# mateomarin/two_towers

Hardware: AMD Instinct MI355X
Metric: training pairs/sec at global batch=8192, 1/2/4/8 GPUs; MRR@10 match (higher is better)
Workload: dtype bf16; 1 GPU; BASELINE configs[2]: EnhancedTwoTowerModel(300, 256), seq_len 64, batch 8192 per GPU, bf16, hard-negative mining k=5 + margin 0.2, dropout 0.1, Adam; global_batch=8192, seq_len=64, hidden=256, embedding_dim=300, parallelism=dp1, loss=hardneg_margin

## Files before the change

two_towers_amd/csrc/tt_gemm.hip:

```cpp
#include <float.h>
#include <stdarg.h>
#include <stdlib.h>

#include <atomic>
#include <type_traits>

#include "tt_api.h"
#include "tt_gemm_core.h"

namespace tt {
static thread_local char g_err[512];
void set_error(const char* fmt, ...) {
  va_list ap;
  va_start(ap, fmt);
  vsnprintf(g_err, sizeof(g_err), fmt, ap);
  va_end(ap);
}
}

namespace tt {
namespace {
struct OptDef {
  const char* name;
  const char* env;
// ... 109 lines not shown
  using ML = std::conditional_t<
      DMA,
      std::conditional_t<TBM == 256 && TBN == 256 && WGM == 2 && WGN == 4,
                         ttg::Loop8<T, AKO, BKO, TT_GEMM_BAL, A3, false, BUF>,
                         ttg::DLoop<T, AKO, BKO, TBM, TBN, WGM, WGN>>,
      ttg::MainLoop<T, AKO, BKO, TBM, TBN>>;
  static_assert(DMA || (TBM == 128 && TBN == 128 && WGM == 2 && WGN == 2), "register path is 128x128");
  constexpr int NT = 64 * WGM * WGN;
  constexpr int LDSB = ML::LDS_BYTES > 64 * (TBN + 4) * 4 ? ML::LDS_BYTES : 64 * (TBN + 4) * 4;
  __shared__ __attribute__((aligned(16))) char lds[LDSB];
  const int ntn = (g.N + TBN - 1) / TBN, ntm = (g.M + TBM - 1) / TBM;
  const int id = xcd_remap(blockIdx.x, gridDim.x);
  const int bs = id / (ntm * ntn), tile = id - bs * (ntm * ntn);
  const int mt = tile / ntn, nt = tile - mt * ntn;
  const int bi = bs / g.splits, s = bs - bi * g.splits;
  const int m0 = mt * TBM, n0 = nt * TBN;
  const T* A = static_cast<const T*>(g.a[bi]);
  const T* B = static_cast<const T*>(g.b[bi]);

  f32x4 acc[ML::TM][ML::TN];
#pragma unroll
  for (int i = 0; i < ML::TM; ++i)
#pragma unroll
    for (int j = 0; j < ML::TN; ++j) acc[i][j] = f32x4{0.f, 0.f, 0.f, 0.f};

  const int nk = (g.K * (int)sizeof(T) + ttg::KTB - 1) / ttg::KTB;
  const int kt0 = s * g.kt_per_split;
  const int kt1 = min(nk, kt0 + g.kt_per_split);

  constexpr bool L8T = DMA && TBM == 256 && TBN == 256 && WGM == 2 && WGN == 4;
  const bool mm = !L8T || !TT_TAIL_SKIP || __builtin_amdgcn_readfirstlane((int)(m0 + (int)(threadIdx.x >> 8) * 128 < g.M));
  auto lrun = [&](const auto& la, const auto& lb) {
    if constexpr (L8T) ML::run(la, lb, g.K, kt0, kt1, lds, acc, mm);
    else ML::run(la, lb, g.K, kt0, kt1, lds, acc);
  };
  auto run = [&](const auto& la) {
    if constexpr (!BKO) {
      lrun(la, ttg::KCPlain<T>{B, g.ldb, n0, g.N});
    } else if constexpr (SHIFT) {
      lrun(la, ttg::KOShift<T>{B, g.ldb, n0, g.N - n0, g.seq_t, g.bshift[bi]});
    } else {
      lrun(la, ttg::KOPlain<T>{B, g.ldb, n0, g.N - n0});
    }
  };
  if constexpr (AKO) {
    ttg::KOPlain<T> la{A, g.lda, m0, g.M - m0};
    if (g.a_split > 0) {
      la.base1 = static_cast<const T*>(g.a_hi[bi]);
      la.csplit = g.a_split;
    }
    run(la);
  } else {
    run(ttg::KCPlain<T>{A, g.lda, m0, g.M});
  }

#ifdef TT_DIAG
  if (g.force_regstage == 9) {
    float sum = 0.f;
#pragma unroll
    for (int i = 0; i < ML::TM; ++i)
#pragma unroll
      for (int j = 0; j < ML::TN; ++j) sum += acc[i][j][0] + acc[i][j][3];
    if (sum == 12345.f) static_cast<float*>(g.c[bi])[0] = 1.f;
    return;
  }
#endif
  const bool partial = g.splits > 1;
  TO* C = partial ? nullptr : static_cast<TO*>(g.c[bi]);
  float* P = partial ? static_cast<float*>(g.c[bi]) + (long)s * g.part_stride : nullptr;
  const long ldc = partial ? (long)g.N : g.ldc;
  const float* bias = partial ? nullptr : g.bias[bi];
  const int wave = threadIdx.x >> 6, lane = threadIdx.x & 63, tid = threadIdx.x;
  constexpr int WTM = TBM / WGM, WTN = TBN / WGN;
  const int wm = wave / WGN * WTM, wn = wave % WGN * WTN;
  constexpr int CLD = TBN + 4;
  constexpr int TPR = TBN / 8;
  constexpr int RPP = NT / TPR;
  float* L = reinterpret_cast<float*>(lds);
  const int cg = (tid % TPR) * 8;
  const __amdgpu_buffer_rsrc_t crs = tt_rsrc(partial ? (const void*)P : (const void*)(C + (long)m0 * ldc + n0));
  float bv[8];
#pragma unroll
  for (int e = 0; e < 8; ++e) bv[e] = 0.f;
  if (bias) {
    if (n0 + cg + 8 <= g.N && g.bias_vec_ok) ld8(bias + n0 + cg, bv);
    else
      for (int e = 0; e < 8; ++e)
        if (n0 + cg + e < g.N) bv[e] = bias[n0 + cg + e];
  }
  for (int hf = 0; hf < TBM / 64; ++hf) {
    if (wm <= hf * 64 && hf * 64 < wm + WTM) {
      const int i0 = (hf * 64 - wm) / 16;
#pragma unroll
      for (int i = 0; i < ML::TM; ++i)
        if (i >= i0 && i < i0 + 4)
#pragma unroll
          for (int j = 0; j < ML::TN; ++j)
#pragma unroll
            for (int r = 0; r < 4; ++r)
              L[(16 * (i - i0) + 4 * (lane >> 4) + r) * CLD + wn + 16 * j + (lane & 15)] = acc[i][j][r];
    }
    __syncthreads();
#pragma unroll
    for (int k = 0; k < 64 / RPP; ++k) {
      const int rl = tid / TPR + RPP * k;
      const int gm = m0 + hf * 64 + rl, gn = n0 + cg;
      if (gm < g.M && gn < g.N) {
        float v[8];
#pragma unroll
        for (int e = 0; e < 8; ++e) v[e] = L[rl * CLD + cg + e];
        const bool full = gn + 8 <= g.N && g.vec_ok;
        if (partial) {
          float* dst = P + (long)gm * ldc + gn;
          if (full) st8(dst, v);
          else
            for (int e = 0; e < 8 && gn + e < g.N; ++e) dst[e] = v[e];
        } else {
#pragma unroll
          for (int e = 0; e < 8; ++e) {
            float x = v[e] * g.alpha + bv[e];
            if (g.relu) x = fmaxf(x, 0.f);
            if (g.drop_thresh) x *= tt_dropout_scale(g.drop_seed, g.drop_row0 + (uint32_t)gm, gn + e, g.drop_thresh, g.drop_inv_keep);
            v[e] = x;
          }
          TO* dst = C + (long)gm * ldc + gn;
          if (full) {
            if (g.beta) {
              float o[8];
              ld8(dst, o);
#pragma unroll
              for (int e = 0; e < 8; ++e) v[e] += o[e];
            }
            if (g.stream_out)
              st8_sc1(crs, (int)(((long)(gm - m0) * ldc + (gn - n0)) * (long)sizeof(TO)), v, (TO*)nullptr);
            else
              st8(dst, v);
          } else {
            for (int e = 0; e < 8 && gn + e < g.N; ++e) {
              float x = v[e];
              if (g.beta) x += Elt<TO>::ld(dst + e);
              Elt<TO>::st(dst + e, x);
            }
          }
        }
      }
    }
    __syncthreads();
  }
}

template <typename TO>
constexpr int EPI_STORES = sizeof(TO) == 2 ? 16 : 32;

template <typename TO, int MI = -1, int NI = -1>
TT_DEV void epi_direct(const GemmArgs& g, const f32x4 (&acc)[8][4], TO* C, const float* bias, int m0, int n0,
                       int wm, int wn, bool full) {
  constexpr int I0 = MI < 0 ? 0 : 4 * MI, I1 = MI < 0 ? 8 : 4 * MI + 4;
  constexpr int JP0 = NI < 0 ? 0 : NI, JP1 = NI < 0 ? 2 : NI + 1;
  const int lane = threadIdx.x & 63, q = lane >> 4, lr = lane & 15;
  float bv[4][4];
#pragma unroll
  for (int j = 0; j < 4; ++j)
#pragma unroll
    for (int e = 0; e < 4; ++e) bv[j][e] = 0.f;
  if (bias) {
#pragma unroll
    for (int j = 2 * JP0; j < 2 * JP1; ++j) {
      const int c = n0 + wn + 16 * j + 4 * q;
      if (full && g.bias_vec_ok) {
        const float4 b4 = *reinterpret_cast<const float4*>(bias + c);
        bv[j][0] = b4.x; bv[j][1] = b4.y; bv[j][2] = b4.z; bv[j][3] = b4.w;
      } else {
        for (int e = 0; e < 4; ++e)
          if (c + e < g.N) bv[j][e] = bias[c + e];
      }
    }
  }
#ifdef TT_DIAG
  if (g.force_regstage == 9) {
    float sum = 0.f;
#pragma unroll
    for (int i = 0; i < 8; ++i)
#pragma unroll
      for (int j = 0; j < 4; ++j) sum += acc[i][j][0] + acc[i][j][3] + bv[j][0];
    if (sum == 12345.f) C[0] = (TO)0;
    return;
  }
#endif
  const __amdgpu_buffer_rsrc_t crs = tt_rsrc(C + (long)m0 * g.ldc + n0);
  auto fin = [&](float x, float b, int gm, int gn) {
    x = x * g.alpha + b;
    if (g.relu) x = fmaxf(x, 0.f);
    if (g.drop_thresh) x *= tt_dropout_scale(g.drop_seed, g.drop_row0 + (uint32_t)gm, gn, g.drop_thresh, g.drop_inv_keep);
    return x;
  };
  auto put = [&](int gm, int gn, uint4 v) {
#ifdef TT_DIAG
    if (g.force_regstage == 10) {
      *reinterpret_cast<uint4*>(C + (long)(gm & 63) * g.ldc + gn) = v;
      return;
    }
#endif
    const int off = (int)(((long)(gm - m0) * g.ldc + (gn - n0)) * (long)sizeof(TO));
    if (g.stream_out == 2) st16_buf_aux<2>(crs, off, v);
    else if (g.stream_out == 3) st16_buf_aux<17>(crs, off, v);
    else if (g.stream_out) st16_sc1(crs, off, v);
    else *reinterpret_cast<uint4*>(C + (long)gm * g.ldc + gn) = v;
  };
#pragma unroll
  for (int i = I0; i < I1; ++i) {
    const int gm = m0 + wm + 16 * i + lr;
    if constexpr (sizeof(TO) == 2) {
#if TT_EPI_PAIR
      if (NI < 0 && full) {
        uint4 v[2];
#pragma unroll
        for (int jp = 0; jp < 2; ++jp) {
          uint32_t w[2][2];
#pragma unroll
          for (int h = 0; h < 2; ++h) {
            const int j = 2 * jp + h, c = n0 + wn + 16 * j + 4 * q;
            float x[4];
#pragma unroll
            for (int e = 0; e < 4; ++e) x[e] = fin(acc[i][j][e], bv[j][e], gm, c + e);
            w[h][0] = (uint32_t)f2bf(x[0]) | ((uint32_t)f2bf(x[1]) << 16);
            w[h][1] = (uint32_t)f2bf(x[2]) | ((uint32_t)f2bf(x[3]) << 16);
          }
          const auto s0 = __builtin_amdgcn_permlane16_swap(w[0][0], w[1][0], false, false);
          const auto s1 = __builtin_amdgcn_permlane16_swap(w[0][1], w[1][1], false, false);
          v[jp] = make_uint4(s0[0], s1[0], s0[1], s1[1]);
        }
        uint4 da, db;
        row_pair(v[0], v[1], da, db);
        const int ra = m0 + wm + 16 * i + (lr & 7);
        const int cs = n0 + wn + 16 * (q & 1) + 8 * (q >> 1) + (lr & 8 ? 32 : 0);
        put(ra, cs, da);
        put(ra + 8, cs, db);
        continue;
      }
#endif
#pragma unroll
      for (int jp = JP0; jp < JP1; ++jp) {
        uint32_t w[2][2];
#pragma unroll
        for (int h = 0; h < 2; ++h) {
          const int j = 2 * jp + h, c = n0 + wn + 16 * j + 4 * q;
          float v[4];
#pragma unroll
          for (int e = 0; e < 4; ++e) v[e] = fin(acc[i][j][e], bv[j][e], gm, c + e);
          w[h][0] = (uint32_t)f2bf(v[0]) | ((uint32_t)f2bf(v[1]) << 16);
          w[h][1] = (uint32_t)f2bf(v[2]) | ((uint32_t)f2bf(v[3]) << 16);
        }
        const auto s0 = __builtin_amdgcn_permlane16_swap(w[0][0], w[1][0], false, false);
        const auto s1 = __builtin_amdgcn_permlane16_swap(w[0][1], w[1][1], false, false);
        const uint4 v = make_uint4(s0[0], s1[0], s0[1], s1[1]);
        const int cs = n0 + wn + 16 * (2 * jp + (q & 1)) + 8 * (q >> 1);
        if (full) {
          put(gm, cs, v);
        } else if (gm < g.M) {
          if (cs + 8 <= g.N && g.vec_ok) {
            put(gm, cs, v);
          } else {
            const uint32_t u[4] = {v.x, v.y, v.z, v.w};
            for (int e = 0; e < 8 && cs + e < g.N; ++e)
              Elt<TO>::st(C + (long)gm * g.ldc + cs + e, __uint_as_float(e & 1 ? u[e >> 1] & 0xFFFF0000u : u[e >> 1] << 16));
          }
        }
      }
    } else {
#pragma unroll
      for (int j = 2 * JP0; j < 2 * JP1; ++j) {
        const int c = n0 + wn + 16 * j + 4 * q;
        float v[4];
#pragma unroll
        for (int e = 0; e < 4; ++e) v[e] = fin(acc[i][j][e], bv[j][e], gm, c + e);
        const uint4 u = make_uint4(__float_as_uint(v[0]), __float_as_uint(v[1]), __float_as_uint(v[2]),
                                   __float_as_uint(v[3]));
        if (full) {
          put(gm, c, u);
        } else if (gm < g.M) {
          if (c + 4 <= g.N && g.vec_ok) put(gm, c, u);
          else
            for (int e = 0; e < 4 && c + e < g.N; ++e) Elt<TO>::st(C + (long)gm * g.ldc + c + e, v[e]);
        }
      }
    }
  }
}

template <int MI, int NI>
TT_DEV void epi_quad_simple(const GemmArgs& g, const f32x4 (&acc)[8][4], bf16_t* C, const float* bias, int m0, int n0,
                            int wm, int wn) {
  const int lane = threadIdx.x & 63, q = lane >> 4, lr = lane & 15;
  float bv[2][4];
#pragma unroll
  for (int h = 0; h < 2; ++h) {
    const float4 b4 = bias ? *reinterpret_cast<const float4*>(bias + n0 + wn + 16 * (2 * NI + h) + 4 * q)
                           : make_float4(0.f, 0.f, 0.f, 0.f);
    bv[h][0] = b4.x; bv[h][1] = b4.y; bv[h][2] = b4.z; bv[h][3] = b4.w;
  }
  const __amdgpu_buffer_rsrc_t crs = tt_rsrc(C + (long)m0 * g.ldc + n0);
  const int cs = wn + 16 * (2 * NI + (q & 1)) + 8 * (q >> 1);
#pragma unroll
  for (int i = 4 * MI; i < 4 * MI + 4; ++i) {
    uint32_t w[2][2];
#pragma unroll
    for (int h = 0; h < 2; ++h) {
      const f32x4 a = acc[i][2 * NI + h];
      w[h][0] = (uint32_t)f2bf(a[0] + bv[h][0]) | ((uint32_t)f2bf(a[1] + bv[h][1]) << 16);
      w[h][1] = (uint32_t)f2bf(a[2] + bv[h][2]) | ((uint32_t)f2bf(a[3] + bv[h][3]) << 16);
    }
    const auto s0 = __builtin_amdgcn_permlane16_swap(w[0][0], w[1][0], false, false);
    const auto s1 = __builtin_amdgcn_permlane16_swap(w[0][1], w[1][1], false, false);
    const uint4 v = make_uint4(s0[0], s1[0], s0[1], s1[1]);
    const int off = (int)(((long)(wm + 16 * i + lr) * g.ldc + cs) * 2L);
    if (g.stream_out == 2) st16_buf_aux<2>(crs, off, v);
    else if (g.stream_out) st16_sc1(crs, off, v);
    else st16_buf(crs, (uint32_t)off, 0, v);
  }
}

TT_DEV float rowgroup_max4(float v) {
  const auto a = __builtin_amdgcn_permlane16_swap(__float_as_uint(v), __float_as_uint(v), false, false);
  v = fmaxf(__uint_as_float(a[0]), __uint_as_float(a[1]));
  const auto b = __builtin_amdgcn_permlane32_swap(__float_as_uint(v), __float_as_uint(v), false, false);
  return fmaxf(__uint_as_float(b[0]), __uint_as_float(b[1]));
}
TT_DEV void epi_chunkmax(const GemmArgs& g, const f32x4 (&acc)[8][4], int m0, int n0, int wm, int wn) {
  const int lane = threadIdx.x & 63, q = lane >> 4, lr = lane & 15;
  const int c0 = n0 + wn;
  const bool masked = (g.label_off >= 0 && g.label_off + m0 + wm < c0 + 64 && c0 < g.label_off + m0 + wm + 128) ||
                      c0 + 64 > g.N;
  float mx[8];
#pragma unroll
  for (int i = 0; i < 8; ++i) {
    float v[16];
#pragma unroll
    for (int j = 0; j < 4; ++j)
#pragma unroll
      for (int r = 0; r < 4; ++r) v[4 * j + r] = acc[i][j][r];
    if (masked) {
      const long lab = g.label_off >= 0 ? g.label_off + m0 + wm + 16 * i + lr : -1;
#pragma unroll
      for (int j = 0; j < 4; ++j)
#pragma unroll
        for (int r = 0; r < 4; ++r) {
          const int col = c0 + 16 * j + 4 * q + r;
          if (col == lab) v[4 * j + r] = -1.f;
          if (col >= g.N) v[4 * j + r] = -FLT_MAX;
        }
    }
    float m = fmaxf(fmaxf(v[0], v[1]), v[2]);
#pragma unroll
    for (int e = 3; e < 15; e += 2) m = fmaxf(fmaxf(m, v[e]), v[e + 1]);
    mx[i] = rowgroup_max4(fmaxf(m, v[15]));
  }
  const long chunk = c0 / 64;
  if (chunk >= g.nch) return;
#pragma unroll
  for (int u = 0; u < 2; ++u) {
    const int i = 2 * q + u;
    float m = mx[0];
#pragma unroll
    for (int e = 1; e < 8; ++e) m = i == e ? mx[e] : m;
    const long row = (long)m0 + wm + 16 * i + lr;
    if (row < g.M) g.cm[row * g.nch + chunk] = m;
  }
}

#ifndef BRES_DIAG
#define BRES_DIAG 0
#endif
#ifndef BRES_STORE
#define BRES_STORE 0
#endif
#ifndef BRES_PD
#define BRES_PD 1
#endif
#ifndef BRES_STAG
#define BRES_STAG 0
#endif
constexpr int BR_COLS = 192;
template <int NKS, int RB = 2>
__global__ __launch_bounds__(RB == 2 ? 512 : 256, 1) void gemm_bres(GemmArgs g, int npan, int nbatch) {
  static_assert(RB == 2 || RB == 4, "32- or 64-row wave tiles");
  constexpr int NW = RB == 2 ? 8 : 4;
  constexpr int NT = 64 * NW;
  constexpr int TR = 16 * RB;
  constexpr int NKT = (NKS + 1) / 2;
  constexpr int IMG = BR_COLS * ttg::KTB;
  constexpr int PD = ((BRES_PD && NKS * RB <= 20) || NKS % 2 != 0) ? NKS : NKS / 2;
  __shared__ __attribute__((aligned(16))) char lds[NKT * IMG + BR_COLS * 4];
  float* bias_s = reinterpret_cast<float*>(lds + NKT * IMG);
  const int tid = threadIdx.x, wave = tid >> 6, lane = tid & 63;
  const int ptot = npan * nbatch;
  const int bid = ttg::xcd_remap(blockIdx.x, gridDim.x);
  const int ngrp = gridDim.x / ptot;
  const int gi = bid / ptot, p = bid % ptot;
  const int bi = p / npan, n0 = (p % npan) * BR_COLS;
  const bf16_t* A = static_cast<const bf16_t*>(g.a[bi]);
  const bf16_t* Bm = static_cast<const bf16_t*>(g.b[bi]);
  bf16_t* C = static_cast<bf16_t*>(g.c[bi]);
  const float* bias = g.bias[bi];
  for (int id = tid; id < NKT * BR_COLS * 8; id += NT) {
    const int kt = id / (BR_COLS * 8), rem = id % (BR_COLS * 8), row = rem >> 3, c = rem & 7;
    const int k = kt * 64 + c * 8;
    uint4 v = make_uint4(0, 0, 0, 0);
    if (k < g.K) v = *reinterpret_cast<const uint4*>(Bm + (long)(n0 + row) * g.ldb + k);
    *reinterpret_cast<uint4*>(lds + kt * IMG + ttg::kc_off(row, c)) = v;
  }
  for (int c = tid; c < BR_COLS; c += NT) bias_s[c] = bias ? bias[n0 + c] : 0.f;
  __syncthreads();
  const int mg = ((g.M + ngrp - 1) / ngrp + TR - 1) / TR * TR;
  const int g0 = gi * mg;
  const int ntl = max(0, min(mg, g.M - g0) + TR - 1) / TR;
  const __amdgpu_buffer_rsrc_t ra = tt_rsrc_n(A + (long)g0 * g.lda, g0 < g.M);
  const int lr = lane & 15, q = lane >> 4;
  auto lda_frag = [&](int t, int ks, int rb) {
    const int row = t * TR + rb * 16 + lr;
    const uint32_t off = t < ntl && g0 + row < g.M ? (uint32_t)((row * (int)g.lda + ks * 32 + q * 8) * 2) : 0x80000000u;
    return ld16_buf(ra, off, 0);
  };
  if (BRES_STAG > 0 && wave >= NW / 2) __builtin_amdgcn_s_sleep(BRES_STAG);
  if (TT_PRIO_HALF && wave >= NW / 2) __builtin_amdgcn_s_setprio(1);
  uint4 ar[PD][RB];
  int t = wave;
#pragma unroll
  for (int i = 0; i < PD; ++i)
#pragma unroll
    for (int rb = 0; rb < RB; ++rb) ar[i][rb] = lda_frag(t, i, rb);
  for (; t < ntl; t += NW) {
    f32x4 acc[RB][BR_COLS / 16];
#pragma unroll
    for (int rb = 0; rb < RB; ++rb)
#pragma unroll
      for (int j = 0; j < BR_COLS / 16; ++j) acc[rb][j] = f32x4{0.f, 0.f, 0.f, 0.f};
#pragma unroll
    for (int ks = 0; ks < NKS; ++ks) {
      uint4 a[RB];
#pragma unroll
      for (int rb = 0; rb < RB; ++rb) a[rb] = ar[ks % PD][rb];
#pragma unroll
      for (int rb = 0; rb < RB; ++rb)
        ar[ks % PD][rb] = ks + PD < NKS ? lda_frag(t, ks + PD, rb) : lda_frag(t + NW, ks + PD - NKS, rb);
      const char* img = lds + (ks >> 1) * IMG;
#pragma unroll
      for (int j = 0; j < BR_COLS / 16; ++j) {
        const uint4 fb = ttg::frag<bf16_t, false>(img, 16 * j, ks & 1);
#pragma unroll
        for (int rb = 0; rb < RB; ++rb) acc[rb][j] = ttg::mma<bf16_t>(fb, a[rb], acc[rb][j]);
      }
      __builtin_amdgcn_sched_barrier(0);
    }
#pragma unroll
    for (int rb = 0; rb < RB; ++rb) {
      const int row = t * TR + rb * 16 + lr;
      const bool ok = g0 + row < g.M;
#pragma unroll
      for (int jp = 0; jp < BR_COLS / 32; ++jp) {
        uint32_t w[2][2];
#pragma unroll
        for (int h = 0; h < 2; ++h) {
          const int j = 2 * jp + h;
          const float4 b4 = *reinterpret_cast<const float4*>(bias_s + 16 * j + 4 * q);
          const float v0 = acc[rb][j][0] + b4.x, v1 = acc[rb][j][1] + b4.y;
          const float v2 = acc[rb][j][2] + b4.z, v3 = acc[rb][j][3] + b4.w;
          w[h][0] = (uint32_t)f2bf(v0) | ((uint32_t)f2bf(v1) << 16);
          w[h][1] = (uint32_t)f2bf(v2) | ((uint32_t)f2bf(v3) << 16);
        }
        const auto s0 = __builtin_amdgcn_permlane16_swap(w[0][0], w[1][0], false, false);
        const auto s1 = __builtin_amdgcn_permlane16_swap(w[0][1], w[1][1], false, false);
        const int cs = n0 + 16 * (2 * jp + (q & 1)) + 8 * (q >> 1);
// ... 79 lines not shown
  for (int j = 0; j < WR_CB; ++j) {
    const float4 b4 = bias ? *reinterpret_cast<const float4*>(bias + n0 + 16 * j + 4 * q) : make_float4(0.f, 0.f, 0.f, 0.f);
    bv[j][0] = b4.x; bv[j][1] = b4.y; bv[j][2] = b4.z; bv[j][3] = b4.w;
  }
#pragma unroll
  for (int j = 0; j < WR_CB; ++j)
#pragma unroll
    for (int ks = 0; ks < NKS; ++ks) asm volatile("" : "+v"(wa[j][ks]));
  const __amdgpu_buffer_rsrc_t rc = tt_rsrc(C + (long)g0 * g.ldc);
  for (int t = 0; t < ntl; ++t) {
    if (t == 0) asm volatile("s_waitcnt vmcnt(%0)" ::"n"(NDMA) : "memory");
    else if (t == 1) asm volatile("s_waitcnt vmcnt(%0)" ::"n"(NDMA + WR_EST) : "memory");
    else asm volatile("s_waitcnt vmcnt(%0)" ::"n"(NDMA + 2 * WR_EST) : "memory");
    asm volatile("s_waitcnt lgkmcnt(0)" ::: "memory");
    __builtin_amdgcn_s_barrier();
    if (NDMA) issue(t + 2);
    __builtin_amdgcn_sched_barrier(0);
    const char* slot = lds + (t % WR_NS) * SLOT;
    auto put = [&](int row, int col, uint4 v) {
      const int gr = t * WR_TR + row;
      const uint32_t off = gr < rows ? (uint32_t)(((long)gr * g.ldc + col) * 2) : 0x80000000u;
#if WR_DIAG & 1
      asm volatile("" ::"v"(v.x), "v"(v.y), "v"(v.z), "v"(v.w), "v"(off));
#else
      st16_buf(rc, off, 0, v);
#endif
    };
#pragma unroll
    for (int ps = 0; ps < NPASS; ++ps) {
      const int r0 = ps * 16 * RB;
      f32x4 acc[RB][WR_CB];
#pragma unroll
      for (int rb = 0; rb < RB; ++rb)
#pragma unroll
        for (int j = 0; j < WR_CB; ++j) acc[rb][j] = f32x4{0.f, 0.f, 0.f, 0.f};
      uint4 a[2][RB];
#pragma unroll
      for (int rb = 0; rb < RB; ++rb) a[0][rb] = ttg::frag<bf16_t, false>(slot, r0 + 16 * rb, 0);
#pragma unroll
      for (int ks = 0; ks < NKS; ++ks) {
        if (ks + 1 < NKS) {
#pragma unroll
          for (int rb = 0; rb < RB; ++rb)
            a[(ks + 1) & 1][rb] = ttg::frag<bf16_t, false>(slot + ((ks + 1) >> 1) * IMG, r0 + 16 * rb, (ks + 1) & 1);
        }
#pragma unroll
        for (int rb = 0; rb < RB; ++rb)
#pragma unroll
          for (int j = 0; j < WR_CB; ++j)
            acc[rb][j] = __builtin_amdgcn_mfma_f32_16x16x32_bf16(__builtin_bit_cast(bf16x8v, wa[j][ks]),
                                                                 __builtin_bit_cast(bf16x8v, a[ks & 1][rb]), acc[rb][j], 0, 0, 0);
        __builtin_amdgcn_sched_barrier(0);
      }
      uint32_t w[RB][WR_CB][2];
#pragma unroll
      for (int rb = 0; rb < RB; ++rb)
#pragma unroll
        for (int j = 0; j < WR_CB; ++j) {
          const f32x4 c = acc[rb][j];
          w[rb][j][0] = pack2bf(c[0] + bv[j][0], c[1] + bv[j][1]);
          w[rb][j][1] = pack2bf(c[2] + bv[j][2], c[3] + bv[j][3]);
        }
      auto pair = [&](int rb, int jp) {
        const auto s0 = __builtin_amdgcn_permlane16_swap(w[rb][2 * jp][0], w[rb][2 * jp + 1][0], false, false);
        const auto s1 = __builtin_amdgcn_permlane16_swap(w[rb][2 * jp][1], w[rb][2 * jp + 1][1], false, false);
        return make_uint4(s0[0], s1[0], s0[1], s1[1]);
      };
#pragma unroll
      for (int rb = 0; rb < RB; ++rb) {
        uint4 da, db;
        row_pair(pair(rb, 0), pair(rb, 1), da, db);
        const int row = r0 + 16 * rb + (lr & 7), cs = n0 + 16 * (q & 1) + 8 * (q >> 1) + (lr & 8 ? 32 : 0);
        put(row, cs, da);
        put(row + 8, cs, db);
      }
    }
  }
  asm volatile("s_waitcnt vmcnt(0)" ::: "memory");
}

template <typename T, bool AKO, bool BKO, bool SHIFT, typename TO, bool A3, bool BUF = false, bool HN = false,
          bool IE = false>
__global__ __launch_bounds__(512) void gemm_persist(GemmArgs g, int ntiles) {
  static_assert(!HN || (A3 && !AKO && !BKO && !SHIFT), "the scan epilogue runs on the A3 direct-epilogue form");
  using L8 = ttg::Loop8<T, AKO, BKO, false, A3, A3, BUF>;
  using Piece = typename L8::Piece;
  constexpr int STG = A3 ? 0 : 32 * 256 * 4;
  static_assert(!A3 || 2 * L8::HALF >= 32 * 256 * 4, "staging fits an A slot");
  __shared__ __attribute__((aligned(16))) char lds[L8::LDS_BYTES + STG];
  float* stg = reinterpret_cast<float*>(lds + L8::LDS_BYTES);
  const int nwg = gridDim.x;
  const int w = xcd_remap(blockIdx.x, nwg);
  if (w >= ntiles) return;
  const int G = g.walk_g > 0 ? g.walk_g : (g.N + 255) / 256;
  const int X = g.walk_x > 0 ? g.walk_x : 1;
  const int P = nwg / X, span = ntiles / X;
  const int qbeg = (w / P) * span + w % P;
  const int qstep = P;
  const int qend = (w / P + 1) * span;
  for (int i = 0; i < (w & 3) * g.skew; ++i) __builtin_amdgcn_s_sleep(64);
  const int ntn = (g.N + 255) / 256, ntm = (g.M + 255) / 256;
  const int nk = (g.K * (int)sizeof(T) + ttg::KTB - 1) / ttg::KTB;
  const int wave = threadIdx.x >> 6, lane = threadIdx.x & 63, tid = threadIdx.x;
  const int wr = wave >> 2, bh = (wave & 3) >> 1, bc = (wave & 1) * 64;
  const int wm = wr * 128, wn = (wave & 3) * 64;
  const uint32_t base = __builtin_amdgcn_readfirstlane(ttg::lds_addr_of(lds));

  struct TileId { int bi, m0, n0; };
  auto decode = [&](int q) {
    TileId t;
    const int u = q / G, per = g.nbatch * ntm;
    const int gr = u / per, rr = u - gr * per;
    t.bi = rr / ntm;
    t.m0 = (rr - t.bi * ntm) * 256;
    t.n0 = (gr * G + (q - u * G)) * 256;
    return t;
  };
  auto loader_a = [&](int q) {
    const TileId t = decode(q < qend ? q : 0);
    const T* A = static_cast<const T*>(g.a[t.bi]);
    if constexpr (AKO) {
      ttg::KOPlain<T> la{A, g.lda, t.m0, q < qend ? g.M - t.m0 : 0};
      if (g.a_split > 0) {
        la.base1 = static_cast<const T*>(g.a_hi[t.bi]);
        la.csplit = g.a_split;
      }
      return la;
    } else {
      return ttg::KCPlain<T>{A, g.lda, t.m0, q < qend ? g.M : t.m0};
    }
  };
  auto loader_b = [&](int q) {
    const TileId t = decode(q < qend ? q : 0);
    const T* B = static_cast<const T*>(g.b[t.bi]);
    if constexpr (!BKO) {
      return ttg::KCPlain<T>{B, g.ldb, t.n0, q < qend ? g.N : t.n0};
    } else if constexpr (SHIFT) {
      return ttg::KOShift<T>{B, g.ldb, t.n0, q < qend ? g.N - t.n0 : 0, g.seq_t, g.bshift[t.bi]};
    } else {
      return ttg::KOPlain<T>{B, g.ldb, t.n0, q < qend ? g.N - t.n0 : 0};
    }
  };
#ifdef TT_DIAG
  if constexpr (A3) {
    if (g.force_regstage == 11) {
      f32x4 acc[8][4];
#pragma unroll
      for (int i = 0; i < 8; ++i)
#pragma unroll
        for (int j = 0; j < 4; ++j) acc[i][j] = f32x4{(float)i, (float)j, 1.f, 2.f};
      for (int q = qbeg; q < qend; q += qstep) {
        const TileId t = decode(q);
        const bool full = t.m0 + 256 <= g.M && t.n0 + 256 <= g.N && g.vec_ok;
        epi_direct<TO>(g, acc, static_cast<TO*>(g.c[t.bi]), g.bias[t.bi], t.m0, t.n0, wm, wn, full);
      }
      return;
    }
  }
#endif
  auto la = loader_a(qbeg);
  auto lb = loader_b(qbeg);
  typename L8::template Half<AKO, decltype(la)> pa0, pa1;
  typename L8::template Half<BKO, decltype(lb)> pb0, pb1;
  pa0.init(la, 0, nk, g.K, 0);
  pa1.init(la, 0, nk, g.K, 128);
  pb0.init(lb, 0, nk, g.K, 0);
  pb1.init(lb, 0, nk, g.K, 128);
  if constexpr (A3) {
    pa0.issue(0, base);
    pa1.issue(0, base + L8::HALF);
    pb0.issue(0, base + L8::BOFF);
    pb1.issue(0, base + L8::BOFF + L8::HALF);
    pa0.issue(1, base + 2 * L8::HALF);
    pa1.issue(1, base + 3 * L8::HALF);
    pb0.issue(1, base + L8::BOFF + 2 * L8::HALF);
    pb1.issue(1, base + L8::BOFF + 3 * L8::HALF);
    asm volatile("s_waitcnt vmcnt(8)" ::: "memory");
  } else {
    pa0.issue(0, base);
    pa1.issue(0, base + L8::HALF);
    pb0.issue(0, base + 2 * L8::HALF);
    pb1.issue(0, base + 3 * L8::HALF);
    pb0.issue(1, base + L8::SLOT + 2 * L8::HALF);
    pb1.issue(1, base + L8::SLOT + 3 * L8::HALF);
    asm volatile("s_waitcnt vmcnt(4)" ::: "memory");
  }
  __builtin_amdgcn_s_barrier();
  const bool late = __builtin_amdgcn_readfirstlane(threadIdx.x) >= 256;
  if (TT_PRIO_HALF && late) __builtin_amdgcn_s_setprio(1);
  if (late) __builtin_amdgcn_s_barrier();

  int git = 0;
  int as = 0;
  int ra_off = 0, rb_off = 0;
  bool epi_full = false;
  constexpr bool IEPI = IE && A3 && !HN && PERSIST_BAL && std::is_same<TO, bf16_t>::value;
  f32x4 acc[8][4];
#pragma unroll
  for (int i = 0; i < 8; ++i)
#pragma unroll
    for (int j = 0; j < 4; ++j) acc[i][j] = f32x4{0.f, 0.f, 0.f, 0.f};
  TileId prev_t{0, 0, 0};
  bool have_prev = false;
  auto iepi = [&](auto mi_c, auto ni_c) {
    constexpr int MI = decltype(mi_c)::value, NI = decltype(ni_c)::value;
    if constexpr (IEPI)
      epi_quad_simple<MI, NI>(g, acc, static_cast<bf16_t*>(g.c[prev_t.bi]), g.bias[prev_t.bi], prev_t.m0, prev_t.n0,
                              wm, wn);
#pragma unroll
    for (int i = 4 * MI; i < 4 * MI + 4; ++i)
#pragma unroll
      for (int j = 2 * NI; j < 2 * NI + 2; ++j) acc[i][j] = f32x4{0.f, 0.f, 0.f, 0.f};
  };
  using C0 = std::integral_constant<int, 0>;
  using C1 = std::integral_constant<int, 1>;
  for (int q = qbeg; q < qend; q += qstep) {
    const int qn = q + qstep;
    const TileId cur_t = decode(q);
    if constexpr (!IEPI) {
#pragma unroll
      for (int i = 0; i < 8; ++i)
#pragma unroll
        for (int j = 0; j < 4; ++j) acc[i][j] = f32x4{0.f, 0.f, 0.f, 0.f};
    }
    uint4 fa[2][4], fb[2][4];
    if constexpr (A3) {
      for (int r = 0; r < nk; ++r, ++git) {
        const bool ep = IEPI && r == 0 && have_prev;
        const int an = as == 0 ? 2 : as - 1;
        const int bs = git & 1;
        const char* ia = lds + as * (2 * L8::HALF) + wr * L8::HALF;
        const char* ib = lds + L8::BOFF + bs * (2 * L8::HALF) + bh * L8::HALF;
        const uint32_t anx = base + (uint32_t)an * (2 * L8::HALF);
        const uint32_t bcur = base + L8::BOFF + (uint32_t)bs * (2 * L8::HALF);
        if (r + 2 == nk) {
          la = loader_a(qn);
          pa0.init(la, 0, nk, g.K, 0);
          pa1.init(la, 0, nk, g.K, 128);
          ra_off = nk;
        }
#if PERSIST_BAL
        if constexpr (IEPI)
          if (ep) iepi(C0{}, C0{});
#pragma unroll
        for (int ks = 0; ks < 2; ++ks) {
#pragma unroll
          for (int i = 0; i < 4; ++i) fa[ks][i] = ttg::frag2<T, AKO>(ia, 16 * i, ks);
#pragma unroll
          for (int j = 0; j < 2; ++j) fb[ks][j] = ttg::frag2<T, BKO>(ib, bc + 16 * j, ks);
        }
        pa0.issue(r + 2 - ra_off, anx);
        L8::quad(0, 0, fa, fb, acc);
        if constexpr (IEPI)
          if (ep) iepi(C0{}, C1{});
#pragma unroll
        for (int ks = 0; ks < 2; ++ks)
#pragma unroll
          for (int j = 2; j < 4; ++j) fb[ks][j] = ttg::frag2<T, BKO>(ib, bc + 16 * j, ks);
        pa1.issue(r + 2 - ra_off, anx + L8::HALF);
        L8::quad(0, 1, fa, fb, acc);
        if constexpr (IEPI)
          if (ep) iepi(C1{}, C1{});
#pragma unroll
        for (int ks = 0; ks < 2; ++ks)
#pragma unroll
          for (int i = 0; i < 4; ++i) fa[ks][i] = ttg::frag2<T, AKO>(ia, 64 + 16 * i, ks);
        L8::quad(1, 1, fa, fb, acc);
        if (r + 2 == nk) {
          lb = loader_b(qn);
          pb0.init(lb, 0, nk, g.K, 0);
          pb1.init(lb, 0, nk, g.K, 128);
          rb_off = nk;
        }
        pb0.issue(r + 2 - rb_off, bcur);
        pb1.issue(r + 2 - rb_off, bcur + L8::HALF);
        if constexpr (IEPI)
          if (ep) iepi(C1{}, C0{});
#else
#pragma unroll
        for (int ks = 0; ks < 2; ++ks) {
#pragma unroll
          for (int i = 0; i < 4; ++i) fa[ks][i] = ttg::frag2<T, AKO>(ia, 16 * i, ks);
#pragma unroll
          for (int j = 0; j < 4; ++j) fb[ks][j] = ttg::frag2<T, BKO>(ib, bc + 16 * j, ks);
        }
        pa0.issue(r + 2 - ra_off, anx);
        L8::quad(0, 0, fa, fb, acc);
        pa1.issue(r + 2 - ra_off, anx + L8::HALF);
        L8::quad(0, 1, fa, fb, acc);
        if (r + 2 == nk) {
          lb = loader_b(qn);
          pb0.init(lb, 0, nk, g.K, 0);
          pb1.init(lb, 0, nk, g.K, 128);
          rb_off = nk;
        }
#pragma unroll
        for (int ks = 0; ks < 2; ++ks)
#pragma unroll
          for (int i = 0; i < 4; ++i) fa[ks][i] = ttg::frag2<T, AKO>(ia, 64 + 16 * i, ks);
        pb0.issue(r + 2 - rb_off, bcur);
        L8::quad(1, 1, fa, fb, acc);
        pb1.issue(r + 2 - rb_off, bcur + L8::HALF);
#endif
#ifdef TT_DIAG
        const bool loose = g.force_regstage == 12 && r < 3 && epi_full;
#else
        constexpr bool loose = false;
#endif
        if constexpr (HN) {
          if (r == 0 && epi_full) asm volatile("s_waitcnt vmcnt(10)" ::: "memory");
          else asm volatile("s_waitcnt vmcnt(8)" ::: "memory");
        } else if (IEPI) {
          if (r == 0 && epi_full) {
            if constexpr (EPI_STORES<TO> == 16) asm volatile("s_waitcnt vmcnt(24)" ::: "memory");
            else asm volatile("s_waitcnt vmcnt(40)" ::: "memory");
          } else if (r == 1 && epi_full) {
            if constexpr (EPI_STORES<TO> == 16) asm volatile("s_waitcnt vmcnt(12)" ::: "memory");
            else asm volatile("s_waitcnt vmcnt(16)" ::: "memory");
          } else {
            asm volatile("s_waitcnt vmcnt(8)" ::: "memory");
          }
        } else if ((r == 0 && epi_full) || loose) {
          if constexpr (EPI_STORES<TO> == 16) asm volatile("s_waitcnt vmcnt(24)" ::: "memory");
          else asm volatile("s_waitcnt vmcnt(40)" ::: "memory");
        } else {
          asm volatile("s_waitcnt vmcnt(8)" ::: "memory");
        }
        L8::quad(1, 0, fa, fb, acc);
        as = as == 2 ? 0 : as + 1;
      }
      ra_off -= nk;
      rb_off -= nk;
      if constexpr (HN) {
        epi_chunkmax(g, acc, cur_t.m0, cur_t.n0, wm, wn);
        epi_full = __builtin_amdgcn_readfirstlane((int)(cur_t.m0 + 256 <= g.M && cur_t.n0 + 256 <= 64 * g.nch)) != 0;
        continue;
      }
      const bool full = cur_t.m0 + 256 <= g.M && cur_t.n0 + 256 <= g.N && g.vec_ok;
      if constexpr (IEPI) {
        prev_t = cur_t;
        have_prev = true;
        epi_full = __builtin_amdgcn_readfirstlane((int)full) != 0;
        continue;
      }
      epi_direct<TO>(g, acc, static_cast<TO*>(g.c[cur_t.bi]), g.bias[cur_t.bi], cur_t.m0, cur_t.n0, wm, wn, full);
      epi_full = __builtin_amdgcn_readfirstlane((int)full) != 0;
      continue;
    }
    for (int r = 0; r < (A3 ? 0 : nk); ++r, ++git) {
      const int cs = git & 1;
      const uint32_t cur = base + cs * L8::SLOT, nxt = base + (cs ^ 1) * L8::SLOT;
      const char* ia = lds + cs * L8::SLOT + wr * L8::HALF;
      const char* ib = lds + cs * L8::SLOT + (2 + bh) * L8::HALF;
      if (r + 1 == nk) {
        la = loader_a(qn);
        pa0.init(la, 0, nk, g.K, 0);
        pa1.init(la, 0, nk, g.K, 128);
        ra_off = nk;
      }
#pragma unroll
      for (int ks = 0; ks < 2; ++ks) {
#pragma unroll
        for (int i = 0; i < 4; ++i) fa[ks][i] = ttg::frag2<T, AKO>(ia, 16 * i, ks);
#pragma unroll
        for (int j = 0; j < 4; ++j) fb[ks][j] = ttg::frag2<T, BKO>(ib, bc + 16 * j, ks);
      }
      pa0.issue(r + 1 - ra_off, nxt);
      L8::quad(0, 0, fa, fb, acc);
      pa1.issue(r + 1 - ra_off, nxt + L8::HALF);
      L8::quad(0, 1, fa, fb, acc);
      if (r + 2 == nk) {
        lb = loader_b(qn);
        pb0.init(lb, 0, nk, g.K, 0);
        pb1.init(lb, 0, nk, g.K, 128);
        rb_off = nk;
      }
#pragma unroll
      for (int ks = 0; ks < 2; ++ks)
#pragma unroll
        for (int i = 0; i < 4; ++i) fa[ks][i] = ttg::frag2<T, AKO>(ia, 64 + 16 * i, ks);
      pb0.issue(r + 2 - rb_off, cur + 2 * L8::HALF);
      L8::quad(1, 1, fa, fb, acc);
      pb1.issue(r + 2 - rb_off, cur + 3 * L8::HALF);
      asm volatile("s_waitcnt vmcnt(4)" ::: "memory");
      L8::quad(1, 0, fa, fb, acc);
    }
    ra_off -= nk;
    rb_off -= nk;
    if (!late) __builtin_amdgcn_s_barrier();

    TO* C = static_cast<TO*>(g.c[cur_t.bi]);
    const float* bias = g.bias[cur_t.bi];
    const int m0 = cur_t.m0, n0 = cur_t.n0;
    const int cg = (tid & 31) * 8, rlo = tid >> 5;
    float bv[8];
#pragma unroll
    for (int e = 0; e < 8; ++e) bv[e] = 0.f;
    if (bias) {
      if (n0 + cg + 8 <= g.N && g.bias_vec_ok) ld8(bias + n0 + cg, bv);
      else
        for (int e = 0; e < 8; ++e)
          if (n0 + cg + e < g.N) bv[e] = bias[n0 + cg + e];
    }
    const __amdgpu_buffer_rsrc_t crs = tt_rsrc(C + (long)m0 * g.ldc + n0);
    for (int p = 0; p < 8; ++p) {
      const int i0 = (p * 32 - wm) / 16;
      if (p * 32 >= wm && p * 32 < wm + 128) {
#pragma unroll
        for (int i = 0; i < 8; ++i)
          if (i >= i0 && i < i0 + 2)
#pragma unroll
            for (int j = 0; j < 4; ++j)
#pragma unroll
              for (int rr = 0; rr < 4; ++rr)
                stg[(16 * (i - i0) + 4 * (lane >> 4) + rr) * 256 + wn + 16 * j + (lane & 15)] = acc[i][j][rr];
      }
      asm volatile("s_waitcnt lgkmcnt(0)" ::: "memory");
      __builtin_amdgcn_s_barrier();
#pragma unroll
      for (int k = 0; k < 2; ++k) {
        const int rl = rlo + 16 * k;
        const int gm = m0 + p * 32 + rl, gn = n0 + cg;
        if (gm < g.M && gn < g.N) {
          float v[8];
          const float4 x0 = *reinterpret_cast<const float4*>(stg + rl * 256 + cg);
          const float4 x1 = *reinterpret_cast<const float4*>(stg + rl * 256 + cg + 4);
          v[0] = x0.x; v[1] = x0.y; v[2] = x0.z; v[3] = x0.w; v[4] = x1.x; v[5] = x1.y; v[6] = x1.z; v[7] = x1.w;
#pragma unroll
          for (int e = 0; e < 8; ++e) {
            float x = v[e] * g.alpha + bv[e];
            if (g.relu) x = fmaxf(x, 0.f);
            if (g.drop_thresh) x *= tt_dropout_scale(g.drop_seed, g.drop_row0 + (uint32_t)gm, gn + e, g.drop_thresh, g.drop_inv_keep);
            v[e] = x;
          }
          TO* dst = C + (long)gm * g.ldc + gn;
          if (gn + 8 <= g.N && g.vec_ok) {
            if (g.stream_out)
              st8_sc1(crs, (int)(((long)(gm - m0) * g.ldc + (gn - n0)) * (long)sizeof(TO)), v, (TO*)nullptr);
            else
              st8(dst, v);
          } else {
            for (int e = 0; e < 8 && gn + e < g.N; ++e) Elt<TO>::st(dst + e, v[e]);
          }
        }
      }
      __builtin_amdgcn_s_barrier();
    }
    if (late && qn < qend) __builtin_amdgcn_s_barrier();
  }
  if constexpr (IE && A3 && !HN && PERSIST_BAL && std::is_same<TO, bf16_t>::value) {
    if (have_prev) {
      iepi(C0{}, C0{});
      iepi(C0{}, C1{});
      iepi(C1{}, C1{});
      iepi(C1{}, C0{});
    }
  }
  if constexpr (A3)
    if (!late) __builtin_amdgcn_s_barrier();
  asm volatile("s_waitcnt vmcnt(0)" ::: "memory");
}

template <typename TO, int V>
__global__ __launch_bounds__(256) void splitk_reduce_kernel(const float* ws, long part_stride, int splits,
                                                            int M, int N, GemmArgs g) {
  const int bi = blockIdx.y;
  const float* P = ws + (long)bi * splits * part_stride;
  TO* C = static_cast<TO*>(g.c[bi]);
  const float* bias = g.bias[bi];
  const long total = (long)M * N / V;
  for (long e = (long)blockIdx.x * 256 + threadIdx.x; e < total; e += (long)gridDim.x * 256) {
    float v[V];
    if constexpr (V == 4) {
      float4 a = make_float4(0.f, 0.f, 0.f, 0.f);
      for (int s = 0; s < splits; ++s) {
        const float4 b = reinterpret_cast<const float4*>(P + (long)s * part_stride)[e];
        a.x += b.x;
        a.y += b.y;
        a.z += b.z;
        a.w += b.w;
      }
      v[0] = a.x, v[1] = a.y, v[2] = a.z, v[3] = a.w;
    } else {
      v[0] = 0.f;
      for (int s = 0; s < splits; ++s) v[0] += P[(long)s * part_stride + e];
    }
    const int m = (int)(e * V / N), n0 = (int)(e * V % N);
#pragma unroll
    for (int u = 0; u < V; ++u) {
      float x = v[u] * g.alpha;
      if (bias) x += bias[n0 + u];
      TO* p = C + (long)m * g.ldc + n0 + u;
      if (g.beta) x += Elt<TO>::ld(p);
      Elt<TO>::st(p, x);
    }
  }
}

// ... 502 lines not shown
```

Measured before the change: 154,200 pairs/s.

## Prefetch epilogue bias via buffer loads during last K step and specialize store policy

Measured after the change: 155,200 pairs/s (median of 6 runs). No clear change (+0.6%).

```diff
diff --git a/two_towers_amd/csrc/tt_gemm.hip b/two_towers_amd/csrc/tt_gemm.hip
--- a/two_towers_amd/csrc/tt_gemm.hip
+++ b/two_towers_amd/csrc/tt_gemm.hip
@@ -285,9 +285,45 @@
 template <typename TO>
 constexpr int EPI_STORES = sizeof(TO) == 2 ? 16 : 32;
 
-template <typename TO, int MI = -1, int NI = -1>
-TT_DEV void epi_direct(const GemmArgs& g, const f32x4 (&acc)[8][4], TO* C, const float* bias, int m0, int n0,
-                       int wm, int wn, bool full) {
+struct BiasQ {
+  uint32_t b0 = 0, b1 = 0, b2 = 0, b3 = 0;
+};
+TT_DEV void bias_fetch(BiasQ& z, const float* bias, int c0, int N) {
+  const int lane = threadIdx.x & 63;
+  const uint32_t voff = (uint32_t)(c0 + 16 * (lane & 3) + 4 * (lane >> 4)) * 4u;
+  const ttg::tt_rsrc4 rs = ttg::make_rsrc4(bias, bias ? (uint32_t)N * 4u : 0u);
+  asm volatile(
+      "buffer_load_dword %0, %4, %5, 0 offen\n\t"
+      "buffer_load_dword %1, %4, %5, 0 offen offset:4\n\t"
+      "buffer_load_dword %2, %4, %5, 0 offen offset:8\n\t"
+      "buffer_load_dword %3, %4, %5, 0 offen offset:12"
+      : "+v"(z.b0), "+v"(z.b1), "+v"(z.b2), "+v"(z.b3)
+      : "v"(voff), "s"(rs)
+      : "memory");
+}
+TT_DEV void bias_pin(BiasQ& z) { asm volatile("" : "+v"(z.b0), "+v"(z.b1), "+v"(z.b2), "+v"(z.b3)); }
+template <int J>
+TT_DEV void bias_bcast(const BiasQ& z, float (&bv)[4]) {
+  static_assert(J >= 0 && J < 4, "column block of the wave's 64 columns");
+  bv[0] = __uint_as_float((uint32_t)__builtin_amdgcn_mov_dpp((int)z.b0, J * 0x55 , 0xF, 0xF, false));
+  bv[1] = __uint_as_float((uint32_t)__builtin_amdgcn_mov_dpp((int)z.b1, J * 0x55, 0xF, 0xF, false));
+  bv[2] = __uint_as_float((uint32_t)__builtin_amdgcn_mov_dpp((int)z.b2, J * 0x55, 0xF, 0xF, false));
+  bv[3] = __uint_as_float((uint32_t)__builtin_amdgcn_mov_dpp((int)z.b3, J * 0x55, 0xF, 0xF, false));
+}
+template <int V>
+using IntC = std::integral_constant<int, V>;
+template <int POL>
+TT_DEV void st16_pol(__amdgpu_buffer_rsrc_t r, int off, uint4 v) {
+  if constexpr (POL == 2) st16_buf_aux<2>(r, off, v);
+  else if constexpr (POL == 3) st16_buf_aux<17>(r, off, v);
+  else if constexpr (POL == 1) st16_sc1(r, off, v);
+  else st16_buf(r, (uint32_t)off, 0, v);
+}
+
+template <typename TO, int POL, bool PRE, int MI = -1, int NI = -1>
+TT_DEV void epi_direct(const GemmArgs& g, const f32x4 (&acc)[8][4], TO* C, const BiasQ& bz, const float* bias, int m0,
+                       int n0, int wm, int wn, bool full_rt) {
+  const bool full = POL >= 0 || full_rt;
   constexpr int I0 = MI < 0 ? 0 : 4 * MI, I1 = MI < 0 ? 8 : 4 * MI + 4;
   constexpr int JP0 = NI < 0 ? 0 : NI, JP1 = NI < 0 ? 2 : NI + 1;
   const int lane = threadIdx.x & 63, q = lane >> 4, lr = lane & 15;
@@ -296,7 +332,16 @@
   for (int j = 0; j < 4; ++j)
 #pragma unroll
     for (int e = 0; e < 4; ++e) bv[j][e] = 0.f;
-  if (bias) {
+  if constexpr (PRE) {
+    if constexpr (NI != 1) {
+      bias_bcast<0>(bz, bv[0]);
+      bias_bcast<1>(bz, bv[1]);
+    }
+    if constexpr (NI != 0) {
+      bias_bcast<2>(bz, bv[2]);
+      bias_bcast<3>(bz, bv[3]);
+    }
+  } else if (bias) {
 #pragma unroll
     for (int j = 2 * JP0; j < 2 * JP1; ++j) {
       const int c = n0 + wn + 16 * j + 4 * q;
@@ -335,10 +380,16 @@
     }
 #endif
     const int off = (int)(((long)(gm - m0) * g.ldc + (gn - n0)) * (long)sizeof(TO));
-    if (g.stream_out == 2) st16_buf_aux<2>(crs, off, v);
-    else if (g.stream_out == 3) st16_buf_aux<17>(crs, off, v);
-    else if (g.stream_out) st16_sc1(crs, off, v);
-    else *reinterpret_cast<uint4*>(C + (long)gm * g.ldc + gn) = v;
+    if constexpr (POL > 0) {
+      st16_pol<POL>(crs, off, v);
+    } else if constexpr (POL == 0) {
+      *reinterpret_cast<uint4*>(C + (long)gm * g.ldc + gn) = v;
+    } else {
+      if (g.stream_out == 2) st16_pol<2>(crs, off, v);
+      else if (g.stream_out == 3) st16_pol<3>(crs, off, v);
+      else if (g.stream_out) st16_pol<1>(crs, off, v);
+      else *reinterpret_cast<uint4*>(C + (long)gm * g.ldc + gn) = v;
+    }
   };
 #pragma unroll
   for (int i = I0; i < I1; ++i) {
@@ -422,35 +473,34 @@
 }
 
 template <int MI, int NI>
-TT_DEV void epi_quad_simple(const GemmArgs& g, const f32x4 (&acc)[8][4], bf16_t* C, const float* bias, int m0, int n0,
+TT_DEV void epi_quad_simple(const GemmArgs& g, const f32x4 (&acc)[8][4], bf16_t* C, const BiasQ& bz, int m0, int n0,
                             int wm, int wn) {
   const int lane = threadIdx.x & 63, q = lane >> 4, lr = lane & 15;
   float bv[2][4];
-#pragma unroll
-  for (int h = 0; h < 2; ++h) {
-    const float4 b4 = bias ? *reinterpret_cast<const float4*>(bias + n0 + wn + 16 * (2 * NI + h) + 4 * q)
-                           : make_float4(0.f, 0.f, 0.f, 0.f);
-    bv[h][0] = b4.x; bv[h][1] = b4.y; bv[h][2] = b4.z; bv[h][3] = b4.w;
-  }
+  bias_bcast<2 * NI>(bz, bv[0]);
+  bias_bcast<2 * NI + 1>(bz, bv[1]);
   const __amdgpu_buffer_rsrc_t crs = tt_rsrc(C + (long)m0 * g.ldc + n0);
   const int cs = wn + 16 * (2 * NI + (q & 1)) + 8 * (q >> 1);
-#pragma unroll
-  for (int i = 4 * MI; i < 4 * MI + 4; ++i) {
-    uint32_t w[2][2];
-#pragma unroll
-    for (int h = 0; h < 2; ++h) {
-      const f32x4 a = acc[i][2 * NI + h];
-      w[h][0] = (uint32_t)f2bf(a[0] + bv[h][0]) | ((uint32_t)f2bf(a[1] + bv[h][1]) << 16);
-      w[h][1] = (uint32_t)f2bf(a[2] + bv[h][2]) | ((uint32_t)f2bf(a[3] + bv[h][3]) << 16);
-    }
-    const auto s0 = __builtin_amdgcn_permlane16_swap(w[0][0], w[1][0], false, false);
-    const auto s1 = __builtin_amdgcn_permlane16_swap(w[0][1], w[1][1], false, false);
-    const uint4 v = make_uint4(s0[0], s1[0], s0[1], s1[1]);
-    const int off = (int)(((long)(wm + 16 * i + lr) * g.ldc + cs) * 2L);
-    if (g.stream_out == 2) st16_buf_aux<2>(crs, off, v);
-    else if (g.stream_out) st16_sc1(crs, off, v);
-    else st16_buf(crs, (uint32_t)off, 0, v);
-  }
+  auto rows = [&](auto pol) {
+#pragma unroll
+    for (int i = 4 * MI; i < 4 * MI + 4; ++i) {
+      uint32_t w[2][2];
+#pragma unroll
+      for (int h = 0; h < 2; ++h) {
+        const f32x4 a = acc[i][2 * NI + h];
+        w[h][0] = (uint32_t)f2bf(a[0] + bv[h][0]) | ((uint32_t)f2bf(a[1] + bv[h][1]) << 16);
+        w[h][1] = (uint32_t)f2bf(a[2] + bv[h][2]) | ((uint32_t)f2bf(a[3] + bv[h][3]) << 16);
+      }
+      const auto s0 = __builtin_amdgcn_permlane16_swap(w[0][0], w[1][0], false, false);
+      const auto s1 = __builtin_amdgcn_permlane16_swap(w[0][1], w[1][1], false, false);
+      const uint4 v = make_uint4(s0[0], s1[0], s0[1], s1[1]);
+      const int off = (int)(((long)(wm + 16 * i + lr) * g.ldc + cs) * 2L);
+      st16_pol<decltype(pol)::value>(crs, off, v);
+    }
+  };
+  if (g.stream_out == 2) rows(IntC<2>{});
+  else if (g.stream_out) rows(IntC<1>{});
+  else rows(IntC<0>{});
 }
 
 TT_DEV float rowgroup_max4(float v) {
@@ -836,7 +886,11 @@
       for (int q = qbeg; q < qend; q += qstep) {
         const TileId t = decode(q);
         const bool full = t.m0 + 256 <= g.M && t.n0 + 256 <= g.N && g.vec_ok;
-        epi_direct<TO>(g, acc, static_cast<TO*>(g.c[t.bi]), g.bias[t.bi], t.m0, t.n0, wm, wn, full);
+        BiasQ bz;
+        bias_fetch(bz, g.bias[t.bi], t.n0 + wn, g.N);
+        asm volatile("s_waitcnt vmcnt(0)" ::: "memory");
+        bias_pin(bz);
+        epi_direct<TO, -1, true>(g, acc, static_cast<TO*>(g.c[t.bi]), bz, nullptr, t.m0, t.n0, wm, wn, full);
       }
       return;
     }
@@ -886,11 +940,12 @@
     for (int j = 0; j < 4; ++j) acc[i][j] = f32x4{0.f, 0.f, 0.f, 0.f};
   TileId prev_t{0, 0, 0};
   bool have_prev = false;
+  constexpr bool PRE = A3 && BUF && !HN;
+  BiasQ bz;
   auto iepi = [&](auto mi_c, auto ni_c) {
     constexpr int MI = decltype(mi_c)::value, NI = decltype(ni_c)::value;
     if constexpr (IEPI)
-      epi_quad_simple<MI, NI>(g, acc, static_cast<bf16_t*>(g.c[prev_t.bi]), g.bias[prev_t.bi], prev_t.m0, prev_t.n0,
-                              wm, wn);
+      epi_quad_simple<MI, NI>(g, acc, static_cast<bf16_t*>(g.c[prev_t.bi]), bz, prev_t.m0, prev_t.n0, wm, wn);
 #pragma unroll
     for (int i = 4 * MI; i < 4 * MI + 4; ++i)
 #pragma unroll
@@ -923,6 +978,8 @@
           pa1.init(la, 0, nk, g.K, 128);
           ra_off = nk;
         }
+        if constexpr (PRE)
+          if (r + 1 == nk) bias_fetch(bz, g.bias[cur_t.bi], cur_t.n0 + wn, g.N);
 #if PERSIST_BAL
         if constexpr (IEPI)
           if (ep) iepi(C0{}, C0{});
@@ -998,7 +1055,7 @@
           if (r == 0 && epi_full) {
             if constexpr (EPI_STORES<TO> == 16) asm volatile("s_waitcnt vmcnt(24)" ::: "memory");
             else asm volatile("s_waitcnt vmcnt(40)" ::: "memory");
-          } else if (r == 1 && epi_full) {
+          } else if (r == 1 && epi_full && nk > 2) {
             if constexpr (EPI_STORES<TO> == 16) asm volatile("s_waitcnt vmcnt(12)" ::: "memory");
             else asm volatile("s_waitcnt vmcnt(16)" ::: "memory");
           } else {
@@ -1010,6 +1067,7 @@
         } else {
           asm volatile("s_waitcnt vmcnt(8)" ::: "memory");
         }
+        if constexpr (PRE) bias_pin(bz);
         L8::quad(1, 0, fa, fb, acc);
         as = as == 2 ? 0 : as + 1;
       }
@@ -1027,7 +1085,15 @@
         epi_full = __builtin_amdgcn_readfirstlane((int)full) != 0;
         continue;
       }
-      epi_direct<TO>(g, acc, static_cast<TO*>(g.c[cur_t.bi]), g.bias[cur_t.bi], cur_t.m0, cur_t.n0, wm, wn, full);
+      {
+        TO* C = static_cast<TO*>(g.c[cur_t.bi]);
+        const float* bias = PRE ? nullptr : g.bias[cur_t.bi];
+        if (!full) epi_direct<TO, -1, PRE>(g, acc, C, bz, bias, cur_t.m0, cur_t.n0, wm, wn, false);
+        else if (g.stream_out == 2) epi_direct<TO, 2, PRE>(g, acc, C, bz, bias, cur_t.m0, cur_t.n0, wm, wn, true);
+        else if (g.stream_out == 3) epi_direct<TO, 3, PRE>(g, acc, C, bz, bias, cur_t.m0, cur_t.n0, wm, wn, true);
+        else if (g.stream_out) epi_direct<TO, 1, PRE>(g, acc, C, bz, bias, cur_t.m0, cur_t.n0, wm, wn, true);
+        else epi_direct<TO, 0, PRE>(g, acc, C, bz, bias, cur_t.m0, cur_t.n0, wm, wn, true);
+      }
       epi_full = __builtin_amdgcn_readfirstlane((int)full) != 0;
       continue;
     }
```
